# TheDisorderedOrganization/MonteCarlo

Hardware: AMD Instinct MI355X
Metric: chain-updates/sec (MC sweeps x M) at M=10^7 per MI355X (higher is better)
Workload: dtype f64

## Files before the change

### montecarlo_amd/csrc/amc_internal.h

```cpp
#pragma once

#include "../../include/amc.h"

#include <hip/hip_runtime.h>

#include <dlfcn.h>
#include <time.h>
#include <unistd.h>

#include <algorithm>
#include <cmath>
#include <cstdarg>
#include <cstdio>
#include <cstdlib>
#include <cstring>
#include <map>
#include <mutex>
#include <new>
#include <string>
#include <vector>

#include "amc_kernels.h"

#ifndef AMC_BUILD_ARCH
// ... 177 lines not shown
    ModelSpec model;
    bool f32 = false;
    bool param_f32 = false;
    bool scaled_policy = false;
    bool script_policy = false;
    bool script_dlogq = false;
    int n_params = 1;
    int n_classes = 1;
    int class_of_move[AMC_MAX_MOVES] = {0};
    bool use_rtc = false;
    double* d_x64 = nullptr;
    std::map<std::string, hipFunction_t> rtc_fn;
    std::vector<hipModule_t> rtc_mods;
};

AMC_INTERNAL int grid_for(const amc_handle* h, int64_t n_items, int blocks_per_cu = 0);
AMC_INTERNAL hipError_t wait_stream(hipStream_t stream);
AMC_INTERNAL hipError_t wait_event(hipEvent_t ev);
AMC_INTERNAL int log_form(const amc_handle* h);
AMC_INTERNAL int log_room(amc_handle* h, int* rows);
AMC_INTERNAL int fold_log(amc_handle* h, bool with_ratio = false, int* ratio_rows = nullptr, amc::xs_word* ratio_dst = nullptr);
AMC_INTERNAL hipError_t alloc_counters(amc_handle* h, bool narrow);
AMC_INTERNAL int counter_room(amc_handle* h, const char* who, uint64_t steps);
AMC_INTERNAL amc::SweepArgs make_sweep_args(const amc_handle* h, int32_t n_steps);
AMC_INTERNAL int reduce_sweep_grid(const amc_handle* h);
AMC_INTERNAL int sweep_impl(amc_handle* h, int64_t n_sweeps, bool fuse_reduce, int* grid_out);
AMC_INTERNAL int red_form(const amc_handle* h);
AMC_INTERNAL int red_row_stride(const amc_handle* h, int grid);
AMC_INTERNAL RedTicket* red_next(amc_handle* h);
AMC_INTERNAL int finish_fused_reduce(amc_handle* h, int grid);
AMC_INTERNAL bool reduce_fits_in_grid(const amc_handle* h, int grid);
AMC_INTERNAL int push_params(amc_handle* h, const double* sigma, const double* weight);
AMC_INTERNAL int check_sigma_f32(const char* who, int k, double s);
#define AMC_REFUSE_PARAM_F32(h, who)                                                                                        \
    do {                                                                                                                    \
        if ((h)->param_f32)                                                                                                 \
            return fail(AMC_ERR_STATE, "%s: not available with param_dtype = AMC_DTYPE_F32 (Float32 policy parameters: sweeps only)", (who)); \
    } while (0)
AMC_INTERNAL int pg_resolve(amc_handle* h);
AMC_INTERNAL void comm_release(amc_handle* h);
struct RtcCode { std::vector<char> code; std::string lowered; };
AMC_INTERNAL int validate_potential_expr(const char* expr, const char* what = "custom potential", const char* var = "x");
AMC_INTERNAL int rtc_compile(const ModelSpec& spec, const std::string& inst, const std::string& arch, const AmcKnobs& knobs, const RtcCode** out,
                             std::string* log_out);
AMC_INTERNAL int rtc_function(amc_handle* h, const std::string& inst, hipFunction_t* fn);
AMC_INTERNAL int rtc_launch(amc_handle* h, const std::string& inst, int grid, void** params);
```

### montecarlo_amd/csrc/amc_math.h

```cpp
#pragma once

#ifndef __HIPCC_RTC__
#include <hip/hip_runtime.h>
#include <stdint.h>
#else
typedef unsigned char uint8_t;
typedef unsigned short uint16_t;
typedef int int32_t;
typedef unsigned int uint32_t;
typedef long int64_t;
typedef unsigned long uint64_t;
#endif

#include "amc_tables.h"

namespace amc {

enum : uint32_t { STREAM_INIT = 0, STREAM_METROPOLIS = 1, STREAM_ESTIMATOR = 2 };
enum : uint32_t { DRAW_NORMAL = 0, DRAW_ACCEPT = 1 };

struct u32x4 { uint32_t x, y, z, w; };

__device__ __forceinline__ void stage_math_tables(double* lds, int tid, int nthreads)
{
    for (int i = tid; i < TAB_DOUBLES; i += nthreads) {
        const double v = AMC_MATH_TABLES[i];
        lds[i] = (i >= TAB_LOG_LOGC && i < TAB_SINPI) ? -2.0 * v : v;
    }
    __syncthreads();
}

__device__ __forceinline__ u32x4 philox4x32_10(u32x4 c, uint32_t k0, uint32_t k1)
{
#pragma unroll
    for (int r = 0; r < 10; ++r) {
        const uint64_t m0 = (uint64_t)0xD2511F53u * c.x;
        const uint64_t m1 = (uint64_t)0xCD9E8D57u * c.z;
        u32x4 n;
        n.x = __builtin_amdgcn_bitop3_b32((uint32_t)(m1 >> 32), c.y, k0, 0x96);
        n.y = (uint32_t)m1;
        n.z = __builtin_amdgcn_bitop3_b32((uint32_t)(m0 >> 32), c.w, k1, 0x96);
        n.w = (uint32_t)m0;
        c = n;
        k0 += 0x9E3779B9u;
        k1 += 0xBB67AE85u;
#ifndef AMC_PHILOX_HOISTED_KEYS
        asm volatile("" : "+s"(k0), "+s"(k1));
#endif
    }
    return c;
}

__device__ __forceinline__ u32x4 draw_counter(uint64_t pair, uint64_t t, uint32_t draw, uint32_t stream)
{
    u32x4 c;
    c.x = (uint32_t)t;
    c.y = ((uint32_t)(t >> 32) & 0xFFFFu) | ((draw & 0xFFFu) << 16) | ((stream & 0xFu) << 28);
    c.z = (uint32_t)pair;
    c.w = (uint32_t)(pair >> 32);
    return c;
}

__device__ __forceinline__ double bits_to_binade(uint32_t lo, uint32_t hi, uint32_t expo_hi)
{
    const uint32_t w_hi = __builtin_amdgcn_alignbit(expo_hi, hi, 12);
    const uint32_t w_lo = __builtin_amdgcn_alignbit(hi, lo, 12);
    return __longlong_as_double((long long)(((uint64_t)w_hi << 32) | w_lo));
}

__device__ __forceinline__ double uniform_co(uint32_t lo, uint32_t hi) { return bits_to_binade(lo, hi, 0x3FFu) - 1.0; }
__device__ __forceinline__ double uniform_oc(uint32_t lo, uint32_t hi) { return 2.0 - bits_to_binade(lo, hi, 0x3FFu); }
__device__ __forceinline__ double angle28(uint32_t w)
{
// ... 13 lines not shown
__device__ __forceinline__ double uniform_pick(uint32_t pick12, uint32_t lo)
{
    return (double)(((uint64_t)pick12 << 24) | (uint64_t)(lo & 0xFFFFFFu)) * 0x1.0p-36;
}

__device__ __forceinline__ double exp_core_f64(double x, const double* T)
{
    const double INV_L = 0x1.71547652b82fep+5;
    const double L_HI = 0x1.62e42fee00000p-6;
    const double L_LO = 0x1.a39ef35793c76p-38;
    const double SHIFT = 0x1.8p52;
    const double t = __builtin_fma(x, INV_L, SHIFT);
    const double kd = t - SHIFT;
    const int32_t ki = (int32_t)(uint32_t)(uint64_t)__double_as_longlong(t);
    double r = __builtin_fma(-kd, L_HI, x);
    r = __builtin_fma(-kd, L_LO, r);
    double p = 0x1.6c16c16c16c17p-10;
    p = __builtin_fma(p, r, 0x1.1111111111111p-7);
    p = __builtin_fma(p, r, 0x1.5555555555555p-5);
    p = __builtin_fma(p, r, 0x1.5555555555555p-3);
    p = __builtin_fma(p, r, 0x1.0000000000000p-1);
    p = __builtin_fma(p, r, 1.0);
    p = __builtin_fma(p, r, 1.0);
    const double y = T[TAB_EXP2 + (ki & 31)] * p;
    const int32_t m = ki >> 5;
    const uint64_t yb = (uint64_t)__double_as_longlong(y);
    const uint32_t yh = (uint32_t)(yb >> 32) + ((uint32_t)m << 20);
    return __longlong_as_double((long long)(((uint64_t)yh << 32) | (yb & 0xffffffffull)));
}

__device__ __forceinline__ double exp_f64(double x, const double* T)
{
    double y = exp_core_f64(x, T);
    y = (x < -708.0) ? 0.0 : y;
    y = (x > 709.0) ? __builtin_huge_val() : y;
    y = (x != x) ? x : y;
    return y;
}

__device__ __forceinline__ double log_f64(double x)
{
    const double LN2_HI = 0x1.62e42fee00000p-1;
    const double LN2_LO = 0x1.a39ef35793c76p-33;
    const double x0 = x;
    int64_t k = 0;
    uint64_t ux = (uint64_t)__double_as_longlong(x);
    if (ux < 0x0010000000000000ull) {
// ... 32 lines not shown
    double s1, s2, s3;
    double c1, c2;
};

__device__ __forceinline__ MathK math_k_literal()
{
    return {2.0 * 0x1.5555555555555p-3, -2.0 * 0x1.999999999999ap-3, -2.0 * 0x1.5555555555555p-2,
            0x1.466bc6775aae2p+1, -0x1.4abbce625be53p+2, 0x1.921fb54442d18p+1,
            0x1.03c1f081b5ac4p+2, -0x1.3bd3cc9be45dep+2};
}

__device__ __forceinline__ MathK math_k_pinned()
{
    MathK k = math_k_literal();
    asm volatile("" : "+v"(k.l1), "+v"(k.l2), "+v"(k.l3), "+v"(k.s1), "+v"(k.s2), "+v"(k.s3), "+v"(k.c1), "+v"(k.c2));
    return k;
}

__device__ __forceinline__ double neg2logbm_f64(double u, const double* T, const MathK& mk = math_k_literal())
{
    const double N2_LN2_HI = -2.0 * 0x1.62e42fee00000p-1;
    const double N2_LN2_LO = -2.0 * 0x1.a39ef35793c76p-33;
    const uint64_t ux = (uint64_t)__double_as_longlong(u);
    uint32_t hx = (uint32_t)(ux >> 32);
    int32_t k = (int32_t)(hx >> 20) - 1023;
    hx &= 0x000fffffu;
    const uint32_t i = (hx + 0x95f64u) & 0x100000u;
    k += (int32_t)(i >> 20);
    hx |= i ^ 0x3ff00000u;
    const double m = __longlong_as_double((long long)(((uint64_t)hx << 32) | (ux & 0xffffffffull)));
    const uint32_t idx = ((hx >> 13) & 0xffu) - TAB_LOG_IDX_MIN;
    const double r = __builtin_fma(m, T[TAB_LOG_INVC + idx], -1.0);
    double p = -2.0 * 0x1.2492492492492p-3;
    p = __builtin_fma(p, r, mk.l1);
    p = __builtin_fma(p, r, mk.l2);
    p = __builtin_fma(p, r, 2.0 * 0x1.0000000000000p-2);
    p = __builtin_fma(p, r, mk.l3);
    p = __builtin_fma(p, r, 2.0 * 0x1.0000000000000p-1);
    p = __builtin_fma(p, r, -2.0);
    const double dk = (double)k;
    const double hi = __builtin_fma(dk, N2_LN2_HI, T[TAB_LOG_LOGC + idx]);
    return __builtin_fma(p, r, __builtin_fma(dk, N2_LN2_LO, hi));
}

__device__ __forceinline__ double logbm_f64(double u, const double* T) { return -0.5 * neg2logbm_f64(u, T); }

__device__ __forceinline__ void sincospi_f64(double w, double& sp, double& cp, const double* T,
                                             const MathK& mk = math_k_literal())
{
    const double SHIFT = 0x1.8p52;
    const double t = __builtin_fma(w, 64.0, SHIFT);
    const double nd = t - SHIFT;
    const uint32_t j = (uint32_t)(uint64_t)__double_as_longlong(t) & 127u;
    const double r = __builtin_fma(nd, -0x1.0p-6, w);
    const double z = r * r;
    double ps = -0x1.32d2cce62bd86p-1;
    ps = __builtin_fma(ps, z, mk.s1);
    ps = __builtin_fma(ps, z, mk.s2);
    ps = __builtin_fma(ps, z, mk.s3);
    const double sr = ps * r;
    double pc = -0x1.55d3c7e3cbffap+0;
    pc = __builtin_fma(pc, z, mk.c1);
    pc = __builtin_fma(pc, z, mk.c2);
    const double cr = __builtin_fma(pc, z, 1.0);
    const double S = T[TAB_SINPI + j], C = T[TAB_COSPI + j];
    sp = __builtin_fma(S, cr, C * sr);
    cp = __builtin_fma(C, cr, -(S * sr));
}

__device__ __forceinline__ double sqrt_radius_f64(double a)
{
    const double y = __builtin_amdgcn_rsq(a);
    double g = a * y;
    double h = y * 0.5;
    const double r = __builtin_fma(-h, g, 0.5);
    g = __builtin_fma(g, r, g);
    h = __builtin_fma(h, r, h);
    double d = __builtin_fma(-g, g, a);
    g = __builtin_fma(d, h, g);
    d = __builtin_fma(-g, g, a);
    g = __builtin_fma(d, h, g);
    return __builtin_fmax(g, 0.0);
}

__device__ __forceinline__ void box_muller(u32x4 v, double& z0, double& z1, const double* T, const MathK& mk = math_k_literal())
{
    const double u = uniform_oc(v.x, v.y);
    const double w = angle28(v.w);
// ... 66 lines not shown
```

### montecarlo_amd/csrc/amc_model.h

```cpp
#pragma once

#include "amc_math.h"
#include "amc_xsum.h"

#define AMC_MAX_MOVES 64
#define AMC_MAX_LEARN 8
#ifndef AMC_BLOCK
#define AMC_BLOCK 256
#endif
#define AMC_PAD_DOUBLES (2 * AMC_BLOCK + 8)

namespace amc {

enum { POT_HARMONIC = 0, POT_DOUBLE_WELL = 1, POT_CUSTOM = 2 };

#ifndef AMC_PLAIN_KERNELS
#define AMC_PLAIN_KERNELS 1
#endif
#ifndef AMC_KERNEL_LINKAGE
#define AMC_KERNEL_LINKAGE
#endif

#ifdef AMC_STATE_F32
typedef float real_t;
// ... 398 lines not shown
    const real_t e1 = potential<POT>(x, T);
    p.xn = x + p.delta;
    const real_t e2 = potential<POT>(p.xn, T);
    p.dlogp = ((-e2) * beta) - ((-e1) * beta);
    return p;
}

__device__ __forceinline__ bool accept_exact(real_t delta, real_t dlogp, param_t den, double rden, double logc, double u,
                                             const double* T)
{
#ifdef AMC_PARAM_F32
    (void)rden;
    const double logq = (double)((-(delta * delta)) / den) - logc;
#else
    const double logq = div_by_const((double)(-(delta * delta)), den, rden) - logc;
#endif
    const double arg = ((double)dlogp + logq) - logq;
    const bool c_pos = arg >= 0.0, c_rng = arg >= -708.0, c_exp = exp_core_f64(arg, T) > u;
    return c_pos | (c_rng & c_exp);
}

#define AMC_FILTER_EPS 0x1.0p-16f
struct FilterCmp {
    bool pos, lo, hi;
};

__device__ __forceinline__ FilterCmp accept_filter(real_t dlogp, uint32_t k)
{
    const float t = (float)dlogp;
    const float ex = __builtin_amdgcn_exp2f(__builtin_fmaxf(t, -17.0f) * 0x1.715476p+0f);
    const float kf = (float)k;
    constexpr float SCALE = 4096.0f;
    const float lo1 = __builtin_fmaf(ex, (1.0f - AMC_FILTER_EPS) * SCALE, -1.0f);
    const float hi = ex * ((1.0f + AMC_FILTER_EPS) * SCALE);
    FilterCmp c;
    c.pos = t > 2e-12f;
    c.lo = lo1 > kf;
    c.hi = hi < kf;
    return c;
}

__device__ __forceinline__ FilterCmp accept_filter_arg(double arg, uint32_t k)
{
    const float t = (float)arg;
    const float ex = __builtin_amdgcn_exp2f(__builtin_fmaxf(t, -17.0f) * 0x1.715476p+0f);
    const float kf = (float)k;
    constexpr float SCALE = 4096.0f;
    const float lo1 = __builtin_fmaf(ex, (1.0f - AMC_FILTER_EPS) * SCALE, -1.0f);
    const float hi = ex * ((1.0f + AMC_FILTER_EPS) * SCALE);
    FilterCmp c;
    c.pos = arg >= 0.0;
    c.lo = lo1 > kf;
    c.hi = hi < kf;
    return c;
}
__device__ __forceinline__ bool accept_exact_arg(double arg, double u, const double* T)
{
    const bool c_pos = arg >= 0.0, c_rng = arg >= -708.0, c_exp = exp_core_f64(arg, T) > u;
    return c_pos | (c_rng & c_exp);
}
struct ScriptStep {
    real_t xn, xr;
    double arg;
};

#ifdef AMC_USER_SCALE
template <int POT>
__device__ __forceinline__ ScriptStep mh_scaled(real_t x, real_t beta, double sigma, double z, const double* T)
{
    const double TWO_PI = 0x1.921fb54442d18p+2;
    const double sc = sigma * user_scale(x, T);
    const double sc2 = sc * sc;
    const real_t delta = (real_t)__builtin_fma(sc, z, 0.0);
    const double logq_f = ((double)(-(delta * delta))) / (2.0 * sc2) - log_f64(TWO_PI * sc2) / 2.0;
    const real_t e1 = potential<POT>(x, T);
    const real_t xn = x + delta;
    const real_t e2 = potential<POT>(xn, T);
// ... 62 lines not shown
__device__ __forceinline__ void mh_pair(real2& xv, real_t b0, real_t b1, param_t sg0, param_t sg1, int k0, int k1,
                                        const double* s_tab, MoveExact m1, param_t z0, param_t z1, u32x4 pn, u32x4 pu,
                                        bool have_pu, u32x4 accept_ctr, uint32_t key0, uint32_t key1, const double* T,
                                        unsigned long long force_mask, uint32_t& acc_bits, unsigned long long& m0,
                                        unsigned long long& m1_out, const UserTheta& th1)
{
    const uint32_t a0_12 = spare_accept12(pn, 0), a1_12 = spare_accept12(pn, 1);
#if defined(AMC_USER_SCALE) || defined(AMC_USER_LOGQ)
    {
#ifdef AMC_USER_LOGQ
        const int mk0 = user_move_key(MULTI ? k0 : 0), mk1 = user_move_key(MULTI ? k1 : 0);
        ScriptStep s0, s1;
        if (MULTI && AMC_SIGMA_MEMO) {
            const SigmaArg a0 = {sg0, mt_log_sigma(s_tab, MULTI ? k0 : 0)}, a1 = {sg1, mt_log_sigma(s_tab, MULTI ? k1 : 0)};
            s0 = mh_script<POT>(xv.x, b0, a0, z0, T, mk0, user_theta_lds(mk0), gauss_row_of(mk0, s_tab));
            s1 = mh_script<POT>(xv.y, b1, a1, z1, T, mk1, user_theta_lds(mk1), gauss_row_of(mk1, s_tab));
        } else {
            s0 = mh_script<POT>(xv.x, b0, sg0, z0, T, mk0, MULTI ? user_theta_lds(mk0) : th1, MULTI ? gauss_row_of(mk0, s_tab) : gauss_row_off());
            s1 = mh_script<POT>(xv.y, b1, sg1, z1, T, mk1, MULTI ? user_theta_lds(mk1) : th1, MULTI ? gauss_row_of(mk1, s_tab) : gauss_row_off());
        }
#else
        const ScriptStep s0 = mh_scaled<POT>(xv.x, b0, sg0, z0, T), s1 = mh_scaled<POT>(xv.y, b1, sg1, z1, T);
#endif
        const FilterCmp c0 = accept_filter_arg(s0.arg, a0_12), c1 = accept_filter_arg(s1.arg, a1_12);
        const unsigned long long acc0 = __builtin_amdgcn_ballot_w64(c0.pos | c0.lo), rej0 = __builtin_amdgcn_ballot_w64(c0.hi);
        const unsigned long long acc1 = __builtin_amdgcn_ballot_w64(c1.pos | c1.lo), rej1 = __builtin_amdgcn_ballot_w64(c1.hi);
        const unsigned long long undecided = __builtin_amdgcn_ballot_w64(true) & ~((acc0 | rej0) & (acc1 | rej1));
        bool a0 = c0.pos | c0.lo, a1 = c1.pos | c1.lo;
        if ((undecided | force_mask) != 0ull) {
            if (!have_pu) {
                asm volatile("" : "+v"(accept_ctr.z));
                pu = philox4x32_10(accept_ctr, key0, key1);
            }
            a0 = accept_exact_arg(s0.arg, uniform_accept(a0_12, pu.x, pu.y), T);
            a1 = accept_exact_arg(s1.arg, uniform_accept(a1_12, pu.z, pu.w), T);
        }
        xv.x = a0 ? s0.xn : s0.xr;
        xv.y = a1 ? s1.xn : s1.xr;
        m0 = __builtin_amdgcn_ballot_w64(a0);
        m1_out = __builtin_amdgcn_ballot_w64(a1);
        acc_bits = (a0 ? 1u : 0u) | (a1 ? 0x100u : 0u);
        return;
    }
#endif
    const Proposal p0 = propose<POT>(xv.x, b0, sg0, z0, T), p1 = propose<POT>(xv.y, b1, sg1, z1, T);
    const real_t xr0 = p0.xn + (-p0.delta), xr1 = p1.xn + (-p1.delta);
    const FilterCmp c0 = accept_filter(p0.dlogp, a0_12), c1 = accept_filter(p1.dlogp, a1_12);
#define AMC_B(c) __builtin_amdgcn_ballot_w64(c)
    const unsigned long long acc0 = AMC_B(c0.pos) | AMC_B(c0.lo), rej0 = AMC_B(c0.hi);
    const unsigned long long acc1 = AMC_B(c1.pos) | AMC_B(c1.lo), rej1 = AMC_B(c1.hi);
    const unsigned long long undecided = AMC_B(true) & ~((acc0 | rej0) & (acc1 | rej1));
#undef AMC_B
    if ((undecided | force_mask) != 0ull) {
        if (!have_pu) {
            asm volatile("" : "+v"(accept_ctr.z));
            pu = philox4x32_10(accept_ctr, key0, key1);
        }
        MoveExact e0 = m1, e1 = m1;
        if (MULTI) {
            e0.dn = mt_den(s_tab, k0); e0.lc = s_tab[MT_LOGC * AMC_MAX_MOVES + k0]; e0.rd = s_tab[MT_RDEN * AMC_MAX_MOVES + k0];
            e1.dn = mt_den(s_tab, k1); e1.lc = s_tab[MT_LOGC * AMC_MAX_MOVES + k1]; e1.rd = s_tab[MT_RDEN * AMC_MAX_MOVES + k1];
        }
        const bool a0 = accept_exact(p0.delta, p0.dlogp, e0.dn, e0.rd, e0.lc, uniform_accept(a0_12, pu.x, pu.y), T);
        const bool a1 = accept_exact(p1.delta, p1.dlogp, e1.dn, e1.rd, e1.lc, uniform_accept(a1_12, pu.z, pu.w), T);
        m0 = __builtin_amdgcn_ballot_w64(a0);
        m1_out = __builtin_amdgcn_ballot_w64(a1);
        xv.x = a0 ? p0.xn : xr0;
        xv.y = a1 ? p1.xn : xr1;
        acc_bits = (a0 ? 1u : 0u) | (a1 ? 0x100u : 0u);
    } else {
        const bool a0 = c0.pos | c0.lo, a1 = c1.pos | c1.lo;
        m0 = acc0;
        m1_out = acc1;
        xv.x = a0 ? p0.xn : xr0;
        xv.y = a1 ? p1.xn : xr1;
        acc_bits = (a0 ? 1u : 0u) | (a1 ? 0x100u : 0u);
    }
}

typedef uint32_t u32v4_t __attribute__((ext_vector_type(4)));

typedef uint32_t u32v2_t __attribute__((ext_vector_type(2)));

__device__ __forceinline__ real2 load_pair_block(const real_t* block_base)
{
    const __amdgpu_buffer_rsrc_t r = __builtin_amdgcn_make_buffer_rsrc((void*)block_base, 0, 0x7fffffff, 0x00020000);
    real2 d;
#ifdef AMC_STATE_F32
    const u32v2_t v = __builtin_amdgcn_raw_buffer_load_b64(r, threadIdx.x * 8, 0, 0);
    d.x = __uint_as_float(v.x);
    d.y = __uint_as_float(v.y);
#else
    const u32v4_t v = __builtin_amdgcn_raw_buffer_load_b128(r, threadIdx.x * 16, 0, 0);
    d.x = __longlong_as_double((long long)(((uint64_t)v.y << 32) | v.x));
    d.y = __longlong_as_double((long long)(((uint64_t)v.w << 32) | v.z));
#endif
    return d;
}

// ... 14 lines not shown
```

### montecarlo_amd/csrc/amc_pg.hip

```cpp
#define AMC_KERNEL_LINKAGE static
#include "amc_internal.h"

static int nl_capacity(int n_learn) { return n_learn <= 1 ? 1 : n_learn <= 2 ? 2 : n_learn <= 4 ? 4 : 8; }

namespace amc {
#define AMC_PG_FUSED(POT, NL, BETA)                                                                                     \
    extern template __global__ void pg_estimate_kernel<POT, NL, BETA, 2, RED_FORM_NONE>(const PgArgs, const SweepArgs);   \
    extern template __global__ void pg_estimate_kernel<POT, NL, BETA, 2, RED_FORM_COLS>(const PgArgs, const SweepArgs);   \
    extern template __global__ void pg_estimate_kernel<POT, NL, BETA, 2, RED_FORM_E>(const PgArgs, const SweepArgs);      \
    extern template __global__ void pg_estimate_kernel<POT, NL, BETA, 2, RED_FORM_NONE, true>(const PgArgs, const SweepArgs)
AMC_PG_FUSED(POT_HARMONIC, 1, false);
AMC_PG_FUSED(POT_HARMONIC, 1, true);
AMC_PG_FUSED(POT_HARMONIC, 2, false);
AMC_PG_FUSED(POT_HARMONIC, 2, true);
AMC_PG_FUSED(POT_DOUBLE_WELL, 1, false);
AMC_PG_FUSED(POT_DOUBLE_WELL, 1, true);
AMC_PG_FUSED(POT_DOUBLE_WELL, 2, false);
AMC_PG_FUSED(POT_DOUBLE_WELL, 2, true);
#undef AMC_PG_FUSED
}

namespace {

const char* tf(bool b) { return b ? "true" : "false"; }
// ... 233 lines not shown
            }
        }
        if (!h->pg_tail_valid || std::memcmp(&tl, &h->pg_tail_host, sizeof(tl)) != 0) {
            hipLaunchKernelGGL(amc::pg_tail_store_kernel, dim3(1), dim3(64), 0, h->stream, tl, h->d_pg_tail);
            AMC_HIP(hipGetLastError());
            h->pg_tail_host = tl;
            h->pg_tail_valid = true;
        }
        a.tail = h->d_pg_tail;
    }
    const int nl = nl_capacity(n_learn);
    int sweep = 0;
    if (with_sweep) {
        { const int rcc = counter_room(h, who, 1); if (rcc != AMC_OK) return rcc; }
        if (h->d_log) { int room = 0; const int rcf = log_room(h, &room); if (rcf != AMC_OK) return rcf; }
        sweep = h->K > 1 ? 2 : (h->d_log ? 1 : 3);
    }
    const bool red = reduce && with_sweep;
    PgPlan plan;
    { const int rcp = pg_plan(h, nl, sweep, red, q_batch, &plan); if (rcp != AMC_OK) return rcp; }
    const int grid = plan.grid;
    const bool mid = plan.mid;
    if (grid_out) *grid_out = grid;
    amc::SweepArgs sw = make_sweep_args(h, 1);
    sw.red_stride = red_row_stride(h, grid);
    const int rc = h->use_rtc                                    ? launch_pg_custom(h, a, sw, grid, nl, sweep, red, mid)
                   : (h->potential == AMC_POTENTIAL_DOUBLE_WELL) ? launch_pg<amc::POT_DOUBLE_WELL>(h, a, sw, grid, nl, sweep, red, mid)
                                                                 : launch_pg<amc::POT_HARMONIC>(h, a, sw, grid, nl, sweep, red, mid);
    if (rc != AMC_OK) return rc;
    if (with_sweep) {
        h->t += 1;
        h->t_counted += 1;
        if (h->d_log) h->log_fill += 1;
    }
    if (advance) h->t_est += 1;
    *nl_out = nl;
    return AMC_OK;
}

static int pg_check_call(const amc_handle* h, const char* who, int n_learn, const int* learn_ids, int q_batch)
{
    if (n_learn < 0 || n_learn > AMC_MAX_LEARN) return fail(AMC_ERR_BAD_ARG, "%s: n_learn must be in [0, %d]", who, AMC_MAX_LEARN);
    if (n_learn > 0 && !learn_ids) return fail(AMC_ERR_BAD_ARG, "%s: learn_ids is NULL", who);
    for (int l = 0; l < n_learn; ++l)
        if (learn_ids[l] < 0 || learn_ids[l] >= h->K) return fail(AMC_ERR_BAD_ARG, "%s: learn_ids[%d] = %d out of range", who, l, learn_ids[l]);
    if (q_batch < 1 || q_batch > AMC_MAX_QBATCH || (int64_t)q_batch * n_learn >= 4096)
        return fail(AMC_ERR_BAD_ARG, "%s: q_batch must be in [1, %d] and q_batch*n_learn < 4096", who, AMC_MAX_QBATCH);
// ... 406 lines not shown
```

### montecarlo_amd/csrc/amc_sweep.h

```cpp
#pragma once

#include "amc_wave_sums.h"

namespace amc {

struct SweepArgs {
    real_t* x;
    const real_t* beta_arr;
    uint8_t* log;
    const double* ptab;
    const uint8_t* pick_tab;
    unsigned long long* acc_total;
    int64_t n_chains;
    int64_t m_stride;
    uint64_t pair0;
    uint64_t t0;
    int32_t n_steps;
    int32_t n_moves;
    uint32_t key0, key1;
    double beta;
    xs_word* red_partials;
    int32_t red_stride;
    int32_t red_cols;
    int32_t log_pos;
    int32_t exact_accept;
    int32_t n_slots;
};

struct StepDraws {
    u32x4 normal;
};

__device__ __forceinline__ StepDraws step_draws(const SweepArgs& a, uint64_t pair, uint64_t t)
{
    StepDraws d;
    d.normal = philox4x32_10(draw_counter(pair, t, DRAW_NORMAL, STREAM_METROPOLIS), a.key0, a.key1);
    return d;
}

#define AMC_PICK_CELLS 4096
#define AMC_PICK_OPEN 0xFFu

__device__ __forceinline__ void stage_pick_table(uint8_t* lds, const uint8_t* tab)
{
    for (int i = threadIdx.x; i < AMC_PICK_CELLS / 16; i += AMC_BLOCK)
        reinterpret_cast<uint4*>(lds)[i] = reinterpret_cast<const uint4*>(tab)[i];
}

__device__ __forceinline__ int categorical_walk(const double* s_tab, int K, double r)
{
    int k = 0;
    for (int i = 0; i < K - 1; ++i) k += (s_tab[MT_CUM * AMC_MAX_MOVES + i] <= r) ? 1 : 0;
    return k;
}

#define AMC_PACKED_LOG_MOVES 8
#define AMC_LOG_NONE 0
#define AMC_LOG_PACKED 1
#define AMC_LOG_BYTES 2
// ... 97 lines not shown
            s_tab[MT_RDEN * AMC_MAX_MOVES + i] = a.ptab[PT_RDEN * AMC_MAX_MOVES + i];
            if (AMC_SIGMA_MEMO) mt_set_log_sigma(s_tab, i, log_f64(a.ptab[PT_SIGMA * AMC_MAX_MOVES + i]));
        }
    }
    const param_t sigma1 = (param_t)a.ptab[PT_SIGMA * AMC_MAX_MOVES];
    const param_t den1 = (param_t)a.ptab[PT_DEN * AMC_MAX_MOVES];
    const double logc1 = a.ptab[PT_LOGC * AMC_MAX_MOVES];
    const double rden1 = a.ptab[PT_RDEN * AMC_MAX_MOVES];
    UserTheta th1 = {0.0, 0.0, 0.0, 0.0, 0.0, 0.0};
#ifdef AMC_USER_LOGQ
    if (!MULTI) th1 = user_theta_uniform(a.ptab, 0);
#endif

    const int64_t n_pairs = (a.n_chains + 1) >> 1;
    const int64_t stride = (int64_t)gridDim.x * AMC_BLOCK;
    const int64_t first = (int64_t)blockIdx.x * AMC_BLOCK;
    unsigned long long wave_acc = 0;
    unsigned long long slots_before = 0;
    if (REDUCE && !LOG && !MULTI && threadIdx.x == 0)
        for (int sl = (int)blockIdx.x; sl < a.n_slots; sl += (int)gridDim.x) slots_before += a.acc_total[sl];

    auto load_x = [&](int64_t b) -> real2 { return load_pair_block(a.x + 2 * b); };
    auto load_b = [&](int64_t b) -> real2 { return load_pair_block(a.beta_arr + 2 * b); };
    real2 x_nxt = {(real_t)0.0, (real_t)0.0}, b_nxt = {(real_t)a.beta, (real_t)a.beta};
    if (first < n_pairs) {
        x_nxt = load_x(first);
        if (BETA) b_nxt = load_b(first);
    }
    constexpr bool AHEAD = SINGLE;
    StepDraws dr_nxt = {};
    if (AHEAD && first < n_pairs) dr_nxt = step_draws(a, a.pair0 + (uint64_t)(first + threadIdx.x), a.t0);
#ifdef AMC_USER_LOGQ
    stage_user_theta(a.ptab, MULTI);
#endif
    stage_math_tables(s_math, threadIdx.x, AMC_BLOCK);
    __builtin_amdgcn_s_waitcnt(0x0F70);
    real2 x_done = {(real_t)0.0, (real_t)0.0};
    uint32_t lw_done = 0;
    int64_t base_done = -1;
    int64_t base = first;
    for (; base + stride < n_pairs; base += stride) {
        const int64_t p = base + threadIdx.x;
        real2 xv = x_nxt;
        const real_t b0 = b_nxt.x, b1 = b_nxt.y;
        x_nxt = load_x(base + stride);
        if (BETA) b_nxt = load_b(base + stride);
        if (base_done >= 0) {
            store_pair_block_writethrough(a.x + 2 * base_done, x_done);
            if (LOG && SINGLE) store_log_pair<LOG>(a, a.log_pos, base_done + threadIdx.x, lw_done);
        }
        const StepDraws dr = dr_nxt;
        uint32_t lw = 0;
        pair_steps<POT, MULTI, LOG, SINGLE, AHEAD>(a, xv, b0, b1, a.pair0 + (uint64_t)p, p, true, true, s_tab, s_pick, s_math,
                                                   sigma1, den1, rden1, logc1, wave_acc, lw, &dr, math_k_literal(), th1, s_mathf);
        if (AHEAD) dr_nxt = step_draws(a, a.pair0 + (uint64_t)(p + stride), a.t0);
        if (REDUCE) {
            red_add_pair<POT, RED_E>(red, xv, true, true, s_math, s_red[threadIdx.x >> 6], a.red_cols);
        }
        x_done = xv;
        lw_done = lw;
        base_done = base;
    }
    if (base < n_pairs) {
        const int64_t p = base + threadIdx.x;
        const bool v0 = p < n_pairs;
        const bool v1 = v0 && (2 * p + 1 < a.n_chains);
        real2 xv = x_nxt;
        if (base_done >= 0) {
            store_pair_block_writethrough(a.x + 2 * base_done, x_done);
            if (LOG && SINGLE) store_log_pair<LOG>(a, a.log_pos, base_done + threadIdx.x, lw_done);
        }
        uint32_t lw = 0;
        pair_steps<POT, MULTI, LOG, SINGLE, AHEAD>(a, xv, b_nxt.x, b_nxt.y, a.pair0 + (uint64_t)(v0 ? p : 0), p, v0, v1,
                                                   s_tab, s_pick, s_math, sigma1, den1, rden1, logc1, wave_acc, lw, &dr_nxt, math_k_literal(), th1, s_mathf);
        if (v0) {
            store_pair_block_writethrough(a.x + 2 * base, xv);
            if (LOG && SINGLE) store_log_pair<LOG>(a, a.log_pos, p, lw);
        }
        if (REDUCE) red_add_pair<POT, RED_E>(red, xv, v0, v1, s_math, s_red[threadIdx.x >> 6], a.red_cols);
    }
    if (REDUCE)
        red_finish<POT, RED_E>(red, s_red, a.red_partials + (int64_t)blockIdx.x * a.red_stride, a.red_stride == RED_COMPACT_WORDS, a.red_cols);
    if (!MULTI) {
        __shared__ unsigned long long s_acc[AMC_BLOCK / 64];
        if ((threadIdx.x & 63) == 0) s_acc[threadIdx.x >> 6] = wave_acc;
        __syncthreads();
        if (threadIdx.x == 0) {
            unsigned long long t = 0;
            for (int w = 0; w < AMC_BLOCK / 64; ++w) t += s_acc[w];
            if (REDUCE && !LOG) {
                if (t != 0) __hip_atomic_fetch_add(a.acc_total + blockIdx.x, t, __ATOMIC_RELAXED, __HIP_MEMORY_SCOPE_AGENT);
                a.red_partials[(int64_t)blockIdx.x * a.red_stride + (a.red_stride == RED_COMPACT_WORDS ? (int)RED_COMPACT_SLOT : (int)RED_ROW_SLOT)] =
                    (xs_word)__double_as_longlong((double)(slots_before + t));
            } else if (t != 0) {
                __hip_atomic_fetch_add(a.acc_total + blockIdx.x, t, __ATOMIC_RELAXED, __HIP_MEMORY_SCOPE_AGENT);
            }
// ... 207 lines not shown
```

### montecarlo_amd/csrc/amc_sweeps.hip

```cpp
#define AMC_KERNEL_LINKAGE static
#include "amc_internal.h"

template <int POT, bool MULTI, int LOG, bool SINGLE, int FORM>
int launch_sweep_beta(amc_handle* h, const amc::SweepArgs& a, int grid)
{
    if (h->beta_arr)
        hipLaunchKernelGGL((amc::sweep_kernel<POT, MULTI, LOG, true, SINGLE, FORM>), dim3(grid), dim3(AMC_BLOCK), 0, h->stream, a);
    else
        hipLaunchKernelGGL((amc::sweep_kernel<POT, MULTI, LOG, false, SINGLE, FORM>), dim3(grid), dim3(AMC_BLOCK), 0, h->stream, a);
    AMC_HIP(hipGetLastError());
    return AMC_OK;
}

template <int POT, int FORM>
int launch_sweep_form(amc_handle* h, const amc::SweepArgs& a, int grid)
{
#define AMC_SWEEP(MULTI, LOG)                                                                                                 \
    (a.n_steps == 1 ? launch_sweep_beta<POT, MULTI, LOG, true, FORM>(h, a, grid) : launch_sweep_beta<POT, MULTI, LOG, false, FORM>(h, a, grid))
    if (h->K > 1 && log_form(h) == AMC_LOG_PACKED) return AMC_SWEEP(true, AMC_LOG_PACKED);
    if (h->K > 1) return AMC_SWEEP(true, AMC_LOG_BYTES);
    if (h->counters) return AMC_SWEEP(false, AMC_LOG_PACKED);
    return AMC_SWEEP(false, AMC_LOG_NONE);
#undef AMC_SWEEP
}

template <int POT>
int launch_sweep(amc_handle* h, const amc::SweepArgs& a, int grid, bool reduce)
{
    if (!reduce) return launch_sweep_form<POT, amc::RED_FORM_NONE>(h, a, grid);
    return red_form(h) == amc::RED_FORM_E ? launch_sweep_form<POT, amc::RED_FORM_E>(h, a, grid) : launch_sweep_form<POT, amc::RED_FORM_COLS>(h, a, grid);
}

static const char* tf(bool b) { return b ? "true" : "false"; }

static int launch_sweep_custom(amc_handle* h, amc::SweepArgs& a, int grid, bool reduce)
{
    const bool multi = h->K > 1;
    const std::string inst = "amc::sweep_kernel<" + std::to_string(h->potential) + "," + tf(multi) + "," + std::to_string(log_form(h)) + "," + tf(h->beta_arr) + "," +
                             tf(a.n_steps == 1) + "," + std::to_string(reduce ? red_form(h) : (int)amc::RED_FORM_NONE) + ">";
    void* params[] = {&a};
    return rtc_launch(h, inst, grid, params);
}

amc::SweepArgs make_sweep_args(const amc_handle* h, int32_t n_steps)
{
    amc::SweepArgs a;
    a.x = h->d_x;
    a.beta_arr = h->beta_arr ? h->d_beta : nullptr;
    a.log = h->d_log;
    a.log_pos = h->log_fill;
    a.ptab = h->d_ptab;
    a.pick_tab = h->d_pick;
    a.acc_total = h->d_acc_slots;
    a.n_chains = h->M;
    a.m_stride = h->M_pad;
    a.pair0 = (uint64_t)h->offset >> 1;
    a.t0 = h->t;
    a.n_steps = n_steps;
    a.n_moves = h->K;
    a.key0 = (uint32_t)h->seed;
    a.key1 = (uint32_t)(h->seed >> 32);
    a.beta = h->beta;
    a.red_partials = h->red[(h->red_head + h->red_count) % RED_TICKETS].h_rows;
    a.red_stride = RED_HOST_STRIDE;
    a.red_cols = h->red_cols;
    a.exact_accept = h->knobs.exact_accept ? 1 : 0;
    a.n_slots = h->n_slots;
    return a;
}

int reduce_sweep_grid(const amc_handle* h)
{
    return grid_for(h, (h->M + 1) / 2, h->blocks_per_cu_pg ? h->blocks_per_cu_pg : h->blocks_per_cu_red);
}

int sweep_impl(amc_handle* h, int64_t n_sweeps, bool fuse_reduce, int* grid_out)
{
    AMC_HIP(hipSetDevice(h->device));
    { const int rc = pg_resolve(h); if (rc != AMC_OK) return rc; }
    int64_t remaining = n_sweeps * (int64_t)h->sweepstep;
    const int grid = fuse_reduce ? reduce_sweep_grid(h) : grid_for(h, (h->M + 1) / 2, remaining == 1 ? h->blocks_per_cu_single : 0);
    if (fuse_reduce && grid > h->n_slots) return fail(AMC_ERR_STATE, "sweep_impl: a grid of %d blocks has no rows to leave its callback sums in (%d)", grid, h->n_slots);
    if (grid_out) *grid_out = grid;
    while (remaining > 0) {
        int32_t chunk = remaining > (1 << 20) ? (1 << 20) : (int32_t)remaining;
        if (h->d_log) {
            int room = 0;
            const int rc = log_room(h, &room);
            if (rc != AMC_OK) return rc;
            if (chunk > room) chunk = room;
        }
        { const int rc = counter_room(h, "amc_sweep", (uint64_t)chunk); if (rc != AMC_OK) return rc; }
        amc::SweepArgs a = make_sweep_args(h, chunk);
        a.red_stride = red_row_stride(h, grid);
        const bool last = remaining == chunk;
        const bool reduce = fuse_reduce && last;
        const int rc = h->use_rtc ? launch_sweep_custom(h, a, grid, reduce)
                       : (h->potential == AMC_POTENTIAL_DOUBLE_WELL) ? launch_sweep<amc::POT_DOUBLE_WELL>(h, a, grid, reduce)
                                                                     : launch_sweep<amc::POT_HARMONIC>(h, a, grid, reduce);
        if (rc != AMC_OK) return rc;
        h->t += (uint64_t)chunk;
        h->t_counted += (uint64_t)chunk;
        if (h->d_log) h->log_fill += chunk;
        remaining -= chunk;
    }
    return AMC_OK;
}

extern "C" {

int amc_sweep(amc_handle* h, int64_t n_sweeps)
{
    if (!h) return fail(AMC_ERR_BAD_ARG, "amc_sweep: NULL handle");
    if (n_sweeps < 0) return fail(AMC_ERR_BAD_ARG, "amc_sweep: n_sweeps < 0");
    if (n_sweeps == 0) return AMC_OK;
    return sweep_impl(h, n_sweeps, false, nullptr);
// ... 15 lines not shown
```

Baseline: 344.0 billion.

## Trim sweep kernel: partial-fold Philox round, packed accept filter, precomputed trip counts

Several micro-optimisations land in the sweep kernel. The first Philox round is partly computed with scalar registers, and the math tables are rotated in LDS so the log-table index no longer needs a subtraction. The log range reduction is simplified, and the accept filter handles both chains together with packed f32 math when MULTI is off, dropping the separate positive-delta test. The host also precomputes full rounds and tail pairs per block so the loop uses a trip count instead of 64-bit bound compares, and the pair counter is carried incrementally. Dropping c.pos and removing the fmax clamp may change which proposals the fast filter decides, and extra kernel arguments and lambdas add register pressure.

After: 358.9 billion (median of 6 runs). 1.04x the previous value.

```diff
diff --git a/montecarlo_amd/csrc/amc_internal.h b/montecarlo_amd/csrc/amc_internal.h
--- a/montecarlo_amd/csrc/amc_internal.h
+++ b/montecarlo_amd/csrc/amc_internal.h
@@ -223,7 +223,7 @@
 AMC_INTERNAL int fold_log(amc_handle* h, bool with_ratio = false, int* ratio_rows = nullptr, amc::xs_word* ratio_dst = nullptr);
 AMC_INTERNAL hipError_t alloc_counters(amc_handle* h, bool narrow);
 AMC_INTERNAL int counter_room(amc_handle* h, const char* who, uint64_t steps);
-AMC_INTERNAL amc::SweepArgs make_sweep_args(const amc_handle* h, int32_t n_steps);
+AMC_INTERNAL amc::SweepArgs make_sweep_args(const amc_handle* h, int32_t n_steps, int grid);
 AMC_INTERNAL int reduce_sweep_grid(const amc_handle* h);
 AMC_INTERNAL int sweep_impl(amc_handle* h, int64_t n_sweeps, bool fuse_reduce, int* grid_out);
 AMC_INTERNAL int red_form(const amc_handle* h);
diff --git a/montecarlo_amd/csrc/amc_math.h b/montecarlo_amd/csrc/amc_math.h
--- a/montecarlo_amd/csrc/amc_math.h
+++ b/montecarlo_amd/csrc/amc_math.h
@@ -21,19 +21,33 @@
 
 struct u32x4 { uint32_t x, y, z, w; };
 
+enum { LDS_ROT = TAB_DOUBLES - TAB_COSPI,
+       LDS_COSPI = 0, LDS_EXP2 = TAB_EXP2 + LDS_ROT, LDS_LOG_INVC = TAB_LOG_INVC + LDS_ROT, LDS_LOG_LOGC = TAB_LOG_LOGC + LDS_ROT,
+       LDS_SINPI = TAB_SINPI + LDS_ROT };
+static_assert(LDS_LOG_INVC >= TAB_LOG_IDX_MIN && LDS_SINPI + 128 == TAB_DOUBLES, "LDS layout of the math tables");
+
 __device__ __forceinline__ void stage_math_tables(double* lds, int tid, int nthreads)
 {
     for (int i = tid; i < TAB_DOUBLES; i += nthreads) {
         const double v = AMC_MATH_TABLES[i];
-        lds[i] = (i >= TAB_LOG_LOGC && i < TAB_SINPI) ? -2.0 * v : v;
+        lds[i < TAB_COSPI ? i + LDS_ROT : i - TAB_COSPI] = (i >= TAB_LOG_LOGC && i < TAB_SINPI) ? -2.0 * v : v;
     }
     __syncthreads();
 }
 
-__device__ __forceinline__ u32x4 philox4x32_10(u32x4 c, uint32_t k0, uint32_t k1)
+__device__ __forceinline__ void philox_next_key(uint32_t& k0, uint32_t& k1)
+{
+    k0 += 0x9E3779B9u;
+    k1 += 0xBB67AE85u;
+#ifndef AMC_PHILOX_HOISTED_KEYS
+    asm volatile("" : "+s"(k0), "+s"(k1));
+#endif
+}
+
+__device__ __forceinline__ u32x4 philox_rounds(u32x4 c, uint32_t k0, uint32_t k1, int n_rounds)
 {
 #pragma unroll
-    for (int r = 0; r < 10; ++r) {
+    for (int r = 0; r < n_rounds; ++r) {
         const uint64_t m0 = (uint64_t)0xD2511F53u * c.x;
         const uint64_t m1 = (uint64_t)0xCD9E8D57u * c.z;
         u32x4 n;
@@ -42,13 +56,34 @@
         n.z = __builtin_amdgcn_bitop3_b32((uint32_t)(m0 >> 32), c.w, k1, 0x96);
         n.w = (uint32_t)m0;
         c = n;
-        k0 += 0x9E3779B9u;
-        k1 += 0xBB67AE85u;
-#ifndef AMC_PHILOX_HOISTED_KEYS
-        asm volatile("" : "+s"(k0), "+s"(k1));
-#endif
+        philox_next_key(k0, k1);
     }
     return c;
+}
+
+__device__ __forceinline__ u32x4 philox4x32_10(u32x4 c, uint32_t k0, uint32_t k1) { return philox_rounds(c, k0, k1, 10); }
+
+__device__ __forceinline__ u32x4 philox4x32_10_uniform_xy(u32x4 c, uint32_t k0, uint32_t k1)
+{
+    const uint64_t m0 = (uint64_t)0xD2511F53u * c.x;
+    const uint64_t m1 = (uint64_t)0xCD9E8D57u * c.z;
+    uint32_t sx = c.y ^ k0, sz = (uint32_t)(m0 >> 32) ^ k1, sw = (uint32_t)m0;
+    philox_next_key(k0, k1);
+    sw ^= k1;
+    asm volatile("" : "+s"(sx), "+s"(sz), "+s"(sw));
+    u32x4 n;
+    n.x = (uint32_t)(m1 >> 32) ^ sx;
+    n.y = (uint32_t)m1;
+    n.z = c.w ^ sz;
+    const uint64_t r0 = (uint64_t)0xD2511F53u * n.x;
+    const uint64_t r1 = (uint64_t)0xCD9E8D57u * n.z;
+    u32x4 q;
+    q.x = __builtin_amdgcn_bitop3_b32((uint32_t)(r1 >> 32), n.y, k0, 0x96);
+    q.y = (uint32_t)r1;
+    q.z = (uint32_t)(r0 >> 32) ^ sw;
+    q.w = (uint32_t)r0;
+    philox_next_key(k0, k1);
+    return philox_rounds(q, k0, k1, 8);
 }
 
 __device__ __forceinline__ u32x4 draw_counter(uint64_t pair, uint64_t t, uint32_t draw, uint32_t stream)
@@ -108,7 +143,7 @@
     p = __builtin_fma(p, r, 0x1.0000000000000p-1);
     p = __builtin_fma(p, r, 1.0);
     p = __builtin_fma(p, r, 1.0);
-    const double y = T[TAB_EXP2 + (ki & 31)] * p;
+    const double y = T[LDS_EXP2 + (ki & 31)] * p;
     const int32_t m = ki >> 5;
     const uint64_t yb = (uint64_t)__double_as_longlong(y);
     const uint32_t yh = (uint32_t)(yb >> 32) + ((uint32_t)m << 20);
@@ -187,15 +222,12 @@
     const double N2_LN2_HI = -2.0 * 0x1.62e42fee00000p-1;
     const double N2_LN2_LO = -2.0 * 0x1.a39ef35793c76p-33;
     const uint64_t ux = (uint64_t)__double_as_longlong(u);
-    uint32_t hx = (uint32_t)(ux >> 32);
-    int32_t k = (int32_t)(hx >> 20) - 1023;
-    hx &= 0x000fffffu;
-    const uint32_t i = (hx + 0x95f64u) & 0x100000u;
-    k += (int32_t)(i >> 20);
-    hx |= i ^ 0x3ff00000u;
+    const uint32_t t = (uint32_t)(ux >> 32) + 0x95f64u;
+    const int32_t k = (int32_t)(t >> 20) - 1023;
+    const uint32_t hx = (t & 0x000fffffu) + (0x3ff00000u - 0x95f64u);
     const double m = __longlong_as_double((long long)(((uint64_t)hx << 32) | (ux & 0xffffffffull)));
-    const uint32_t idx = ((hx >> 13) & 0xffu) - TAB_LOG_IDX_MIN;
-    const double r = __builtin_fma(m, T[TAB_LOG_INVC + idx], -1.0);
+    const uint32_t idx = (hx >> 13) & 0xffu;
+    const double r = __builtin_fma(m, T[LDS_LOG_INVC - TAB_LOG_IDX_MIN + idx], -1.0);
     double p = -2.0 * 0x1.2492492492492p-3;
     p = __builtin_fma(p, r, mk.l1);
     p = __builtin_fma(p, r, mk.l2);
@@ -204,7 +236,7 @@
     p = __builtin_fma(p, r, 2.0 * 0x1.0000000000000p-1);
     p = __builtin_fma(p, r, -2.0);
     const double dk = (double)k;
-    const double hi = __builtin_fma(dk, N2_LN2_HI, T[TAB_LOG_LOGC + idx]);
+    const double hi = __builtin_fma(dk, N2_LN2_HI, T[LDS_LOG_LOGC - TAB_LOG_IDX_MIN + idx]);
     return __builtin_fma(p, r, __builtin_fma(dk, N2_LN2_LO, hi));
 }
 
@@ -228,7 +260,7 @@
     pc = __builtin_fma(pc, z, mk.c1);
     pc = __builtin_fma(pc, z, mk.c2);
     const double cr = __builtin_fma(pc, z, 1.0);
-    const double S = T[TAB_SINPI + j], C = T[TAB_COSPI + j];
+    const double S = T[LDS_SINPI + j], C = T[LDS_COSPI + j];
     sp = __builtin_fma(S, cr, C * sr);
     cp = __builtin_fma(C, cr, -(S * sr));
 }
diff --git a/montecarlo_amd/csrc/amc_model.h b/montecarlo_amd/csrc/amc_model.h
--- a/montecarlo_amd/csrc/amc_model.h
+++ b/montecarlo_amd/csrc/amc_model.h
@@ -444,37 +444,44 @@
 
 #define AMC_FILTER_EPS 0x1.0p-16f
 struct FilterCmp {
-    bool pos, lo, hi;
+    bool lo, hi;
 };
 
-__device__ __forceinline__ FilterCmp accept_filter(real_t dlogp, uint32_t k)
-{
-    const float t = (float)dlogp;
-    const float ex = __builtin_amdgcn_exp2f(__builtin_fmaxf(t, -17.0f) * 0x1.715476p+0f);
-    const float kf = (float)k;
-    constexpr float SCALE = 4096.0f;
-    const float lo1 = __builtin_fmaf(ex, (1.0f - AMC_FILTER_EPS) * SCALE, -1.0f);
-    const float hi = ex * ((1.0f + AMC_FILTER_EPS) * SCALE);
-    FilterCmp c;
-    c.pos = t > 2e-12f;
-    c.lo = lo1 > kf;
-    c.hi = hi < kf;
-    return c;
-}
-
-__device__ __forceinline__ FilterCmp accept_filter_arg(double arg, uint32_t k)
-{
-    const float t = (float)arg;
-    const float ex = __builtin_amdgcn_exp2f(__builtin_fmaxf(t, -17.0f) * 0x1.715476p+0f);
-    const float kf = (float)k;
-    constexpr float SCALE = 4096.0f;
-    const float lo1 = __builtin_fmaf(ex, (1.0f - AMC_FILTER_EPS) * SCALE, -1.0f);
-    const float hi = ex * ((1.0f + AMC_FILTER_EPS) * SCALE);
-    FilterCmp c;
-    c.pos = arg >= 0.0;
-    c.lo = lo1 > kf;
-    c.hi = hi < kf;
-    return c;
+typedef float f32x2 __attribute__((ext_vector_type(2)));
+
+template <bool PACKED>
+__device__ __forceinline__ void accept_filter_f32(float t0, float t1, uint32_t k0, uint32_t k1, FilterCmp& c0, FilterCmp& c1)
+{
+    const float kf0 = (float)k0, kf1 = (float)k1;
+    constexpr float LOG2E = 0x1.715476p+0f, SCALE = 4096.0f;
+    constexpr float LO = (1.0f - AMC_FILTER_EPS) * SCALE, HI = (1.0f + AMC_FILTER_EPS) * SCALE;
+    f32x2 lo1, hi;
+    if (PACKED) {
+        const f32x2 y = f32x2{t0, t1} * LOG2E;
+        const f32x2 ex = {__builtin_amdgcn_exp2f(y.x), __builtin_amdgcn_exp2f(y.y)};
+        lo1 = __builtin_elementwise_fma(ex, f32x2{LO, LO}, f32x2{-1.0f, -1.0f});
+        hi = ex * HI;
+    } else {
+        const float e0 = __builtin_amdgcn_exp2f(t0 * LOG2E), e1 = __builtin_amdgcn_exp2f(t1 * LOG2E);
+        lo1 = f32x2{__builtin_fmaf(e0, LO, -1.0f), __builtin_fmaf(e1, LO, -1.0f)};
+        hi = f32x2{e0 * HI, e1 * HI};
+    }
+    c0.lo = lo1.x > kf0;
+    c0.hi = hi.x < kf0;
+    c1.lo = lo1.y > kf1;
+    c1.hi = hi.y < kf1;
+}
+
+template <bool PACKED>
+__device__ __forceinline__ void accept_filter(real_t dlogp0, real_t dlogp1, uint32_t k0, uint32_t k1, FilterCmp& c0, FilterCmp& c1)
+{
+    accept_filter_f32<PACKED>((float)dlogp0, (float)dlogp1, k0, k1, c0, c1);
+}
+
+template <bool PACKED>
+__device__ __forceinline__ void accept_filter_arg(double arg0, double arg1, uint32_t k0, uint32_t k1, FilterCmp& c0, FilterCmp& c1)
+{
+    accept_filter_f32<PACKED>((float)arg0, (float)arg1, k0, k1, c0, c1);
 }
 __device__ __forceinline__ bool accept_exact_arg(double arg, double u, const double* T)
 {
@@ -583,11 +590,12 @@
 #else
         const ScriptStep s0 = mh_scaled<POT>(xv.x, b0, sg0, z0, T), s1 = mh_scaled<POT>(xv.y, b1, sg1, z1, T);
 #endif
-        const FilterCmp c0 = accept_filter_arg(s0.arg, a0_12), c1 = accept_filter_arg(s1.arg, a1_12);
-        const unsigned long long acc0 = __builtin_amdgcn_ballot_w64(c0.pos | c0.lo), rej0 = __builtin_amdgcn_ballot_w64(c0.hi);
-        const unsigned long long acc1 = __builtin_amdgcn_ballot_w64(c1.pos | c1.lo), rej1 = __builtin_amdgcn_ballot_w64(c1.hi);
+        FilterCmp c0, c1;
+        accept_filter_arg<!MULTI>(s0.arg, s1.arg, a0_12, a1_12, c0, c1);
+        const unsigned long long acc0 = __builtin_amdgcn_ballot_w64(c0.lo), rej0 = __builtin_amdgcn_ballot_w64(c0.hi);
+        const unsigned long long acc1 = __builtin_amdgcn_ballot_w64(c1.lo), rej1 = __builtin_amdgcn_ballot_w64(c1.hi);
         const unsigned long long undecided = __builtin_amdgcn_ballot_w64(true) & ~((acc0 | rej0) & (acc1 | rej1));
-        bool a0 = c0.pos | c0.lo, a1 = c1.pos | c1.lo;
+        bool a0 = c0.lo, a1 = c1.lo;
         if ((undecided | force_mask) != 0ull) {
             if (!have_pu) {
                 asm volatile("" : "+v"(accept_ctr.z));
@@ -605,13 +613,25 @@
     }
 #endif
     const Proposal p0 = propose<POT>(xv.x, b0, sg0, z0, T), p1 = propose<POT>(xv.y, b1, sg1, z1, T);
-    const real_t xr0 = p0.xn + (-p0.delta), xr1 = p1.xn + (-p1.delta);
-    const FilterCmp c0 = accept_filter(p0.dlogp, a0_12), c1 = accept_filter(p1.dlogp, a1_12);
+    FilterCmp c0, c1;
+    accept_filter<!MULTI>(p0.dlogp, p1.dlogp, a0_12, a1_12, c0, c1);
 #define AMC_B(c) __builtin_amdgcn_ballot_w64(c)
-    const unsigned long long acc0 = AMC_B(c0.pos) | AMC_B(c0.lo), rej0 = AMC_B(c0.hi);
-    const unsigned long long acc1 = AMC_B(c1.pos) | AMC_B(c1.lo), rej1 = AMC_B(c1.hi);
+    const unsigned long long acc0 = AMC_B(c0.lo), rej0 = AMC_B(c0.hi);
+    const unsigned long long acc1 = AMC_B(c1.lo), rej1 = AMC_B(c1.hi);
     const unsigned long long undecided = AMC_B(true) & ~((acc0 | rej0) & (acc1 | rej1));
 #undef AMC_B
+    auto settle = [&](bool r0, bool r1, bool a0, bool a1) {
+        if (MULTI) {
+            xv.x = r0 ? p0.xn + (-p0.delta) : p0.xn;
+            xv.y = r1 ? p1.xn + (-p1.delta) : p1.xn;
+        } else {
+            xv.x = p0.xn;
+            xv.y = p1.xn;
+            if (r0) { xv.x = p0.xn + (-p0.delta); asm volatile("" : "+v"(xv.x)); }
+            if (r1) { xv.y = p1.xn + (-p1.delta); asm volatile("" : "+v"(xv.y)); }
+        }
+        acc_bits = (a0 ? 1u : 0u) | (a1 ? 0x100u : 0u);
+    };
     if ((undecided | force_mask) != 0ull) {
         if (!have_pu) {
             asm volatile("" : "+v"(accept_ctr.z));
@@ -626,16 +646,11 @@
         const bool a1 = accept_exact(p1.delta, p1.dlogp, e1.dn, e1.rd, e1.lc, uniform_accept(a1_12, pu.z, pu.w), T);
         m0 = __builtin_amdgcn_ballot_w64(a0);
         m1_out = __builtin_amdgcn_ballot_w64(a1);
-        xv.x = a0 ? p0.xn : xr0;
-        xv.y = a1 ? p1.xn : xr1;
-        acc_bits = (a0 ? 1u : 0u) | (a1 ? 0x100u : 0u);
+        settle(!a0, !a1, a0, a1);
     } else {
-        const bool a0 = c0.pos | c0.lo, a1 = c1.pos | c1.lo;
         m0 = acc0;
         m1_out = acc1;
-        xv.x = a0 ? p0.xn : xr0;
-        xv.y = a1 ? p1.xn : xr1;
-        acc_bits = (a0 ? 1u : 0u) | (a1 ? 0x100u : 0u);
+        settle(c0.hi, c1.hi, c0.lo, c1.lo);
     }
 }
 
diff --git a/montecarlo_amd/csrc/amc_pg.hip b/montecarlo_amd/csrc/amc_pg.hip
--- a/montecarlo_amd/csrc/amc_pg.hip
+++ b/montecarlo_amd/csrc/amc_pg.hip
@@ -279,7 +279,7 @@
     const int grid = plan.grid;
     const bool mid = plan.mid;
     if (grid_out) *grid_out = grid;
-    amc::SweepArgs sw = make_sweep_args(h, 1);
+    amc::SweepArgs sw = make_sweep_args(h, 1, 0);
     sw.red_stride = red_row_stride(h, grid);
     const int rc = h->use_rtc                                    ? launch_pg_custom(h, a, sw, grid, nl, sweep, red, mid)
                    : (h->potential == AMC_POTENTIAL_DOUBLE_WELL) ? launch_pg<amc::POT_DOUBLE_WELL>(h, a, sw, grid, nl, sweep, red, mid)
diff --git a/montecarlo_amd/csrc/amc_sweep.h b/montecarlo_amd/csrc/amc_sweep.h
--- a/montecarlo_amd/csrc/amc_sweep.h
+++ b/montecarlo_amd/csrc/amc_sweep.h
@@ -25,6 +25,8 @@
     int32_t log_pos;
     int32_t exact_accept;
     int32_t n_slots;
+    int32_t full_rounds;
+    int32_t tail_pairs;
 };
 
 struct StepDraws {
@@ -34,7 +36,7 @@
 __device__ __forceinline__ StepDraws step_draws(const SweepArgs& a, uint64_t pair, uint64_t t)
 {
     StepDraws d;
-    d.normal = philox4x32_10(draw_counter(pair, t, DRAW_NORMAL, STREAM_METROPOLIS), a.key0, a.key1);
+    d.normal = philox4x32_10_uniform_xy(draw_counter(pair, t, DRAW_NORMAL, STREAM_METROPOLIS), a.key0, a.key1);
     return d;
 }
 
@@ -178,14 +180,17 @@
 
     auto load_x = [&](int64_t b) -> real2 { return load_pair_block(a.x + 2 * b); };
     auto load_b = [&](int64_t b) -> real2 { return load_pair_block(a.beta_arr + 2 * b); };
+    const int trips = a.full_rounds + ((int)(blockIdx.x * AMC_BLOCK) < a.tail_pairs ? 1 : 0);
     real2 x_nxt = {(real_t)0.0, (real_t)0.0}, b_nxt = {(real_t)a.beta, (real_t)a.beta};
-    if (first < n_pairs) {
+    if (trips > 0) {
         x_nxt = load_x(first);
         if (BETA) b_nxt = load_b(first);
     }
+    uint64_t pair = a.pair0 + (uint64_t)(first + threadIdx.x);
+    asm volatile("" : "+v"(pair));
     constexpr bool AHEAD = SINGLE;
     StepDraws dr_nxt = {};
-    if (AHEAD && first < n_pairs) dr_nxt = step_draws(a, a.pair0 + (uint64_t)(first + threadIdx.x), a.t0);
+    if (AHEAD && trips > 0) dr_nxt = step_draws(a, pair, a.t0);
 #ifdef AMC_USER_LOGQ
     stage_user_theta(a.ptab, MULTI);
 #endif
@@ -195,8 +200,7 @@
     uint32_t lw_done = 0;
     int64_t base_done = -1;
     int64_t base = first;
-    for (; base + stride < n_pairs; base += stride) {
-        const int64_t p = base + threadIdx.x;
+    for (int full = trips - 1; full > 0; --full, base += stride) {
         real2 xv = x_nxt;
         const real_t b0 = b_nxt.x, b1 = b_nxt.y;
         x_nxt = load_x(base + stride);
@@ -207,9 +211,10 @@
         }
         const StepDraws dr = dr_nxt;
         uint32_t lw = 0;
-        pair_steps<POT, MULTI, LOG, SINGLE, AHEAD>(a, xv, b0, b1, a.pair0 + (uint64_t)p, p, true, true, s_tab, s_pick, s_math,
+        pair_steps<POT, MULTI, LOG, SINGLE, AHEAD>(a, xv, b0, b1, pair, base + threadIdx.x, true, true, s_tab, s_pick, s_math,
                                                    sigma1, den1, rden1, logc1, wave_acc, lw, &dr, math_k_literal(), th1, s_mathf);
-        if (AHEAD) dr_nxt = step_draws(a, a.pair0 + (uint64_t)(p + stride), a.t0);
+        pair += (uint64_t)stride;
+        if (AHEAD) dr_nxt = step_draws(a, pair, a.t0);
         if (REDUCE) {
             red_add_pair<POT, RED_E>(red, xv, true, true, s_math, s_red[threadIdx.x >> 6], a.red_cols);
         }
@@ -217,7 +222,7 @@
         lw_done = lw;
         base_done = base;
     }
-    if (base < n_pairs) {
+    if (trips > 0) {
         const int64_t p = base + threadIdx.x;
         const bool v0 = p < n_pairs;
         const bool v1 = v0 && (2 * p + 1 < a.n_chains);
@@ -227,7 +232,7 @@
             if (LOG && SINGLE) store_log_pair<LOG>(a, a.log_pos, base_done + threadIdx.x, lw_done);
         }
         uint32_t lw = 0;
-        pair_steps<POT, MULTI, LOG, SINGLE, AHEAD>(a, xv, b_nxt.x, b_nxt.y, a.pair0 + (uint64_t)(v0 ? p : 0), p, v0, v1,
+        pair_steps<POT, MULTI, LOG, SINGLE, AHEAD>(a, xv, b_nxt.x, b_nxt.y, v0 ? pair : a.pair0, p, v0, v1,
                                                    s_tab, s_pick, s_math, sigma1, den1, rden1, logc1, wave_acc, lw, &dr_nxt, math_k_literal(), th1, s_mathf);
         if (v0) {
             store_pair_block_writethrough(a.x + 2 * base, xv);
diff --git a/montecarlo_amd/csrc/amc_sweeps.hip b/montecarlo_amd/csrc/amc_sweeps.hip
--- a/montecarlo_amd/csrc/amc_sweeps.hip
+++ b/montecarlo_amd/csrc/amc_sweeps.hip
@@ -42,7 +42,7 @@
     return rtc_launch(h, inst, grid, params);
 }
 
-amc::SweepArgs make_sweep_args(const amc_handle* h, int32_t n_steps)
+amc::SweepArgs make_sweep_args(const amc_handle* h, int32_t n_steps, int grid)
 {
     amc::SweepArgs a;
     a.x = h->d_x;
@@ -66,6 +66,12 @@
     a.red_cols = h->red_cols;
     a.exact_accept = h->knobs.exact_accept ? 1 : 0;
     a.n_slots = h->n_slots;
+    a.full_rounds = a.tail_pairs = 0;
+    if (grid > 0) {
+        const int64_t n_pairs = (h->M + 1) / 2, round = (int64_t)grid * AMC_BLOCK;
+        a.full_rounds = (int32_t)(n_pairs / round);
+        a.tail_pairs = (int32_t)(n_pairs % round);
+    }
     return a;
 }
 
@@ -82,6 +88,8 @@
     const int grid = fuse_reduce ? reduce_sweep_grid(h) : grid_for(h, (h->M + 1) / 2, remaining == 1 ? h->blocks_per_cu_single : 0);
     if (fuse_reduce && grid > h->n_slots) return fail(AMC_ERR_STATE, "sweep_impl: a grid of %d blocks has no rows to leave its callback sums in (%d)", grid, h->n_slots);
     if (grid_out) *grid_out = grid;
+    if (h->knobs.debug_plan)
+        std::fprintf(stderr, "[amc] sweep: %lld pairs in a grid of %d blocks, %lld pairs per round\n", (long long)((h->M + 1) / 2), grid, (long long)grid * AMC_BLOCK);
     while (remaining > 0) {
         int32_t chunk = remaining > (1 << 20) ? (1 << 20) : (int32_t)remaining;
         if (h->d_log) {
@@ -91,7 +99,7 @@
             if (chunk > room) chunk = room;
         }
         { const int rc = counter_room(h, "amc_sweep", (uint64_t)chunk); if (rc != AMC_OK) return rc; }
-        amc::SweepArgs a = make_sweep_args(h, chunk);
+        amc::SweepArgs a = make_sweep_args(h, chunk, grid);
         a.red_stride = red_row_stride(h, grid);
         const bool last = remaining == chunk;
         const bool reduce = fuse_reduce && last;
```
